# apschera2023uzk/MWR_fast_forward_operators_and_LBLs

Hardware: AMD Instinct MI355X
Metric: TB evaluations/sec (profile x channel x angle) (higher is better)
Workload: dtype f64

## Files before the change

mwr_fast_forward_operators_and_lbls_amd/csrc/mwrt_absorption.hip.h:

```cpp
#pragma once
#include "mwrt_math.hip.h"

namespace mwrt {

typedef const __attribute__((address_space(4))) LineMasks* cmasks;
__device__ __forceinline__ LineMasks load_masks(const LineMasks* table, int chunk) {
  const cmasks q = (cmasks)table + chunk;
  LineMasks lm;
  lm.o2_far = q->o2_far; lm.h2o_far = q->h2o_far; lm.h2o_none = q->h2o_none; lm.h2o_res = q->h2o_res; lm.h2o_sd = q->h2o_sd;
  lm.h2o_sdfar = q->h2o_sdfar; lm.h2o_sdint = q->h2o_sdint;
  lm.h2o_vfar = q->h2o_vfar; lm.o2_vfar = q->o2_vfar; lm.vf_u0 = q->vf_u0; lm.vf_h = q->vf_h; lm.vf_invh = q->vf_invh;
  return lm;
}

struct LevelState {
  double t;
  double p;
  double rho;
  double pdry;
};

__device__ __forceinline__ double goff_gratch_e(double tk, double rh) {
  const double LN10 = 2.302585092994045684;
  const double INV_LN10 = 0.434294481903251828;
// ... 122 lines not shown
  }
}
template <int NFC>
__device__ __forceinline__ void far_group_close(const double (&N)[NFC], const double (&D)[NFC], double (&sum)[NFC]) {
  double r[NFC];
#pragma unroll
  for (int j = 0; j < NFC; ++j) r[j] = __builtin_amdgcn_rcp(D[j]);
#pragma unroll
  for (int j = 0; j < NFC; ++j) r[j] = __builtin_fma(r[j], __builtin_fma(-D[j], r[j], 1.0), r[j]);
#pragma unroll
  for (int j = 0; j < NFC; ++j) sum[j] = N[j] * r[j];
}
template <int NFC, class Mask, class Setup>
__device__ __forceinline__ void far_groups_accumulate(const double* sfq, Mask m, Setup&& setup, double (&sum)[NFC]) {
  auto next_quad = [&](FarLine (&q)[4]) {
#pragma unroll
    for (int i = 0; i < 4; ++i) { setup(__builtin_ctzll((unsigned long long)m), q[i]); m &= m - Mask(1); }
    LDS_RELOAD_FENCE();
  };
  while (m) {
    double N[NFC], D[NFC];
    {
      FarLine q[4];
      next_quad(q);
      far_quad_fraction<NFC, true>(sfq, q[0], q[1], q[2], q[3], sum, N, D);
    }
    for (int g = 1; g < FAR_GROUP_QUADS && m; ++g) {
      FarLine q[4];
      next_quad(q);
      far_quad_fraction<NFC, false>(sfq, q[0], q[1], q[2], q[3], sum, N, D);
    }
    far_group_close<NFC>(N, D, sum);
  }
}

constexpr int VF_TERMS = 8;
__device__ __forceinline__ void vfar_add(const FarLine& fl, double u0, double h, double (&acc)[VF_TERMS]) {
  const double d0 = __builtin_fma(u0, u0 + fl.A2, fl.Bc);
  const double d1h = __builtin_fma(fl.A2, h, (2.0 * u0) * h);
  double rd = __builtin_amdgcn_rcp(d0);
  rd = __builtin_fma(rd, __builtin_fma(-d0, rd, 1.0), rd);
  const double a = -d1h * rd, b = (-(h * h)) * rd;
  double cm2 = __builtin_fma(fl.P, u0, fl.Q) * rd;
  double cm1 = __builtin_fma(a, cm2, (fl.P * h) * rd);
  acc[0] += cm2;
  acc[1] += cm1;
#pragma unroll
  for (int j = 2; j < VF_TERMS; ++j) {
    const double cj = __builtin_fma(a, cm1, b * cm2);
    acc[j] += cj;
    cm2 = cm1; cm1 = cj;
  }
}
template <int NFC>
__device__ __forceinline__ void vfar_eval(const double* sfq, double invh, double mu , const double (&acc)[VF_TERMS], double (&sum)[NFC]) {
  constexpr int G = (NFC % 7 == 0) ? 7 : ((NFC % 4 == 0) ? 4 : 2);
  static_assert(NFC % G == 0, "group width");
#pragma unroll
  for (int j0 = 0; j0 < NFC; j0 += G) {
    double x[G], p[G];
#pragma unroll
    for (int g = 0; g < G; ++g) { x[g] = __builtin_fma(sfq[2 * (j0 + g) + 1], invh, mu); p[g] = acc[VF_TERMS - 1]; }
#pragma unroll
    for (int k = VF_TERMS - 2; k >= 0; --k) {
#pragma unroll
      for (int g = 0; g < G; ++g) p[g] = __builtin_fma(p[g], x[g], acc[k]);
// ... 268 lines not shown
        if (wave_any(inner)) {
          const double r1 = inner ? sd_shape(d1) - q.base : 0.0;
          sum[j] = __builtin_fma(q.s, r1, sum[j]);
        }
      }
    }
  }
  const bool dry = !(L.rho > 0.0);
#pragma unroll
  for (int j = 0; j < NFC; ++j) {
    const double f2 = sfq[2 * j + 1];
    awet[j] = dry ? 0.0 : (3.183e-05 * den * sum[j] + con0) * f2;
  }
}

template <bool FUSED>
__device__ __forceinline__ double table_addend(double s) {
  if constexpr (FUSED) {
    double v;
    asm("v_mov_b64 %0, %1" : "=v"(v) : "s"(s));
    return v;
  } else {
    return s;
  }
}

struct O2Line {
  double c1, df2;
  double P, Q;
  double cc;
  double dnu;
};

template <int NFC, bool NODES = false, bool GROUPED = false>
__device__ __forceinline__ void dry_absorb(cmodel M, const LevelState& L, const double* sfq ,
                                           const LineMasks& lm, double (&adry)[NFC], unsigned long long excl = 0ull,
                                           const double* init_sum = nullptr, unsigned long long* failed = nullptr) {
  const double temp = L.t;
  const double pres = L.p;
  const double th = fdiv(300.0, temp);
  const double th1 = th - 1.0;
  const double lnth = flog(th);
  const double b = fexp(M->o2_x * lnth);
  const double preswv = fdiv(L.rho * temp, M->o2_pvap_div);
  const double presda = pres - preswv;
  const double den = 0.001 * (presda * b + M->o2_wv_factor * preswv * th);
  const double dens = 0.001 * (presda + M->o2_wv_factor * preswv) * th;
  const double dfnr = M->o2_wb300 * den;
  const double pe2 = den * den;
  const bool second = M->o2_mix_mode != 0;
  const double ymul = second ? den : 0.001 * pres * b;
  const bool line1_dens = !second && M->o2_line1_dens;

  double sum[NFC];
#pragma unroll
  for (int j = 0; j < NFC; ++j) sum[j] = init_sum ? init_sum[j] : 0.0;

  long long be_prev = -1;
  double ebe = 1.0;
  auto line_setup = [&](int k) -> O2Line {
    const auto& R = M->o2r[k];
    if constexpr (GROUPED) asm volatile("" :: "s"(R.be), "s"(R.w300), "s"(R.y0), "s"(R.y1));
    const double y = ymul * __builtin_fma(R.y1, th1, table_addend<GROUPED>(R.y0));
    double dnu = 0.0, gfac = 1.0;
    if (second) {
      dnu = pe2 * __builtin_fma(R.dnu1, th1, table_addend<GROUPED>(R.dnu0));
      gfac = __builtin_fma(pe2, __builtin_fma(R.g1, th1, table_addend<GROUPED>(R.g0)), 1.0);
    }
    const double df = R.w300 * ((k == 0 && line1_dens) ? dens : den);
    const long long be_bits = __builtin_bit_cast(long long, R.be);
    if (be_bits != be_prev) { ebe = fexp(-R.be * th1); be_prev = be_bits; }
    const double str = R.s300rf2 * ebe;
    O2Line q;
    q.dnu = dnu;
    q.c1 = R.f + dnu;
    q.df2 = df * df;
    const double a = (str * df) * gfac;
    const double cb = q.c1 * (str * y);
    q.cc = __builtin_fma(q.c1, q.c1, q.df2);
    q.P = a + cb;
    q.Q = q.cc * (a - cb);
    return q;
  };

  const int nl = M->n_o2;
  const unsigned long long all = o2_lines_all(nl) & ~excl;
  unsigned long long near = ~lm.o2_far & all;
  const unsigned long long setA = (MWRT_ABLATE & 1) ? 0ull : o2_far_set(lm, all);
  const unsigned long long setV = o2_vfar_set(lm, setA, NODES);
  const unsigned long long setQ = o2_quad_set(lm, setA, NODES);
  const unsigned long long leftA = lowest_bits(setQ, __builtin_popcountll(setQ) & 3);
  const unsigned long long leftP = (__builtin_popcountll(leftA) >= 2) ? lowest_bits(leftA, 2) : 0ull;
  near |= leftA & ~leftP;
  auto far_setup = [&](int k, FarLine& fl) {
    const O2Line q = line_setup(k);
    double P = q.P, Q = q.Q;
    if (!NODES && second && !wave_all(fabs(q.dnu) < FAR_SHIFT_GHZ)) { near |= 1ull << k; P = 0.0; Q = 0.0; }
    fl.P = P; fl.Q = Q;
    fl.A2 = 2.0 * __builtin_fma(-q.c1, q.c1, q.df2);
    fl.Bc = q.cc * q.cc;
  };
  if (setV) {
    double acc[VF_TERMS];
#pragma unroll
    for (int j = 0; j < VF_TERMS; ++j) acc[j] = 0.0;
    for (unsigned long long m = setV; m; m &= m - 1ull) {
      FarLine q;
      far_setup(__builtin_ctzll(m), q);
      vfar_add(q, lm.vf_u0, lm.vf_h, acc);
    }
    LDS_RELOAD_FENCE();
    vfar_eval<NFC>(sfq, lm.vf_invh, -lm.vf_u0 * lm.vf_invh, acc, sum);
  }
  if constexpr (GROUPED) far_groups_accumulate<NFC>(sfq, setQ & ~leftA, far_setup, sum);
  else for (unsigned long long m = setQ & ~leftA; m;) {
    FarLine q0, q1, q2, q3;
    far_setup(__builtin_ctzll(m), q0); m &= m - 1ull;
    far_setup(__builtin_ctzll(m), q1); m &= m - 1ull;
    far_setup(__builtin_ctzll(m), q2); m &= m - 1ull;
    far_setup(__builtin_ctzll(m), q3); m &= m - 1ull;
    LDS_RELOAD_FENCE();
    far_quad_accumulate<NFC>(sfq, q0, q1, q2, q3, sum);
  }
  if (leftP) {
    FarLine q0, q1;
    unsigned long long m = leftP;
    far_setup(__builtin_ctzll(m), q0); m &= m - 1ull;
    far_setup(__builtin_ctzll(m), q1);
    LDS_RELOAD_FENCE();
    far_pair_accumulate<NFC>(sfq, q0, q1, sum);
  }
  if (MWRT_ABLATE & 1) near = 0ull;
  be_prev = -1;
  for (unsigned long long m = near; m; m &= m - 1ull) {
    const int k = __builtin_ctzll(m);
    const O2Line q = line_setup(k);
    LDS_RELOAD_FENCE();
#pragma unroll
    for (int j = 0; j < NFC; ++j) {
      const double f = sfq[2 * j], f2 = sfq[2 * j + 1];
      const double d1 = f - q.c1;
      const double d2 = f + q.c1;
      const double D1 = __builtin_fma(d1, d1, q.df2);
      const double D2 = __builtin_fma(d2, d2, q.df2);
      const double den12 = D1 * D2;
// ... 129 lines not shown
```

mwr_fast_forward_operators_and_lbls_amd/csrc/mwrt_fused.hip.h:

```cpp
#pragma once
#include "mwrt_absorption.hip.h"
#include "mwrt_layer.hip.h"

namespace mwrt {

__device__ __forceinline__ void blank_outputs(const FusedArgs& A, int64_t prof, int jbase, int nfc, int tid, int nthreads) {
  const double qnan = __builtin_nan("");
  const int nang = A.nang, nlev = A.nlev;
  for (int it = tid; it < nfc * nang; it += nthreads) {
    const int j = it / nang, a = it % nang;
    const int64_t o = (prof * nang + a) * A.nf + jbase + j;
    A.tb[o] = qnan;
    if (A.tbatm) A.tbatm[o] = qnan;
    if (A.tmr) A.tmr[o] = qnan;
    if (A.tauwet) A.tauwet[o] = qnan;
    if (A.taudry) A.taudry[o] = qnan;
    if (A.tauliq) A.tauliq[o] = qnan;
    if (A.tauice) A.tauice[o] = qnan;
  }
  if (A.taulay) for (int it = tid; it < nfc * nlev; it += nthreads)
    A.taulay[(prof * A.nf + jbase + it / nlev) * nlev + it % nlev] = qnan;
}

typedef const __attribute__((address_space(3))) double* ldoubles;
template <class Step>
__device__ __forceinline__ void rte_segment(const double* tau_seg, const double* bof_seg, int seglen, Step step) {
  ldoubles tp = (ldoubles)tau_seg, bp = (ldoubles)bof_seg;
  asm volatile("" : "+v"(tp), "+v"(bp));
  double t0 = tp[0], t1 = tp[1], b0 = bp[0], b1 = bp[1];
  for (int n = seglen >> 2; n > 0; --n) {
    const double t2 = tp[2], t3 = tp[3];
    step(t0, b0);
    const double b2 = bp[2], b3 = bp[3];
    step(t1, b1);
    t0 = tp[4]; t1 = tp[5];
    step(t2, b2);
    b0 = bp[4]; b1 = bp[5];
    step(t3, b3);
    tp += 4; bp += 4;
  }
  const int rest = seglen & 3;
  if (rest > 0) step(t0, b0);
  if (rest > 1) step(t1, b1);
  if (rest > 2) step(tp[2], bp[2]);
}

template <int NFC, int NFK, int MAXT, bool OPT = false, bool EXTRAS = false, bool ALPHA = false>
__global__ void __launch_bounds__(MAXT, (MAXT <= 256 ? (EXTRAS ? MWRT_MIN_WAVES : (ALPHA ? 4 : 3)) : 1))
k_tb_fused(const FusedArgs A) {
  constexpr int NPASS = (NFC + NFK - 1) / NFK;
  static_assert(NPASS <= 2, "LaunchGeom carries the split of two passes");
  extern __shared__ __attribute__((aligned(16))) double lds[];
  const int tid = threadIdx.x;
  const int lane = tid & (WAVE - 1);
  const int wave = tid / WAVE;
  const int nthreads = blockDim.x;
  const int nwaves = nthreads / WAVE;
  const int64_t prof = blockIdx.x;
  const int mi = (int)(prof / A.nprof_in);
  const int64_t pin = prof - mi * A.nprof_in;
  const int jbase = blockIdx.y * NFC;
  const int nfc = min(NFC, A.nf - jbase);
  const int nlev = A.nlev, nang = A.nang, ld = A.g.ldrow;
  const cmodel M = (cmodel)A.Ms[mi];
  const cdoubles cfrq = (cdoubles)A.frq;
  const cdoubles cam = (cdoubles)A.airmass;

  double* tau = lds;
  double* bof = tau + (size_t)NFK * ld;
  double* part = bof + (size_t)NFK * ld;
  double* scratch = part + (size_t)A.g.npart;
  double* edge = scratch + 16;
  auto row = [&](int j) -> double* { return (j < NFK ? tau + (size_t)j * ld : bof + (size_t)(j - NFK) * ld); };
  constexpr bool GROUPED = MAXT <= 512;
  constexpr bool PARK = !ALPHA && GROUPED;
  constexpr int GRP = 16;
  const int ngrp = nthreads / GRP;
// ... 49 lines not shown
      for (int j = 0; j < NFC; ++j) { awet[j] = 0.0; adry[j] = 0.0; }
    }
    if (active && bad) atomicOr(&s_flag, 1);
  }
  double denl = 0.0, deni = 0.0, o3n = 0.0;
  if constexpr (OPT) {
    if (A.denliq) denl = A.denliq[off];
    if (A.denice) deni = A.denice[off];
    if (A.o3n) o3n = A.o3n[off];
    if (active && (isnan(denl) || isnan(deni) || isnan(o3n))) atomicOr(&s_flag, 1);
  }
  __syncthreads();
  if (s_flag) {
    blank_outputs(A, prof, jbase, nfc, tid, nthreads);
    if (tid == 0) A.valid[prof] = 0;
    return;
  }

  if constexpr (!ALPHA) {
    const double e = goff_gratch_e(ti, rhi);
    const LevelState L = level_state(pi, ti, e);
    const LineMasks lm = load_masks(A.masks[mi], blockIdx.y);
    MWRT_STAMP(1);
    MWRT_SETPRIO(3);
    h2o_absorb<NFC, false, GROUPED>(M, L, sfq, lm, awet);
    if constexpr (PARK) {
      if (active) {
#pragma unroll
        for (int j = 0; j < NFC; ++j) row(j)[tid] = awet[j];
      }
    }
    MWRT_STAMP(2);
    MWRT_SETPRIO(2);
    dry_absorb<NFC, false, GROUPED>(M, L, sfq, lm, adry);
    MWRT_SETPRIO(1);
    MWRT_STAMP(3);
    if constexpr (OPT) {
      if (A.o3n) {
        LDS_RELOAD_FENCE();
        x_absorb<NFC>(M, A.t[off], A.p[off], A.o3n[off], sfq, adry);
      }
    }
  }
  if (lane == WAVE - 1) {
#pragma unroll
    for (int j = 0; j < NFC; ++j) {
      if constexpr (!PARK) edge[wave * 2 * NFC + j] = awet[j];
      edge[wave * 2 * NFC + NFC + j] = adry[j];
    }
  }
  __syncthreads();
  if constexpr (OPT) { LDS_RELOAD_FENCE(); zi = A.z[off]; ti = A.t[off]; }
  double tw[EXTRAS ? NFC : 1], td[NFC];
  bool neg = false;
  {
    const double z0 = A.z[pin * nlev];
    const double dz = (active && tid > 0) ? ((zi - z0) - (A.z[off - 1] - z0)) : 0.0;
    const bool seam = (lane == 0) && (wave > 0);
    const bool has_prev = active && tid > 0;
    [[maybe_unused]] ldoubles wrow = nullptr;
    [[maybe_unused]] double pw_next = 0.0, aw_next = 0.0;
    if constexpr (PARK) {
      wrow = (ldoubles)(tau + (has_prev ? tid - 1 : 0));
      asm volatile("" : "+v"(wrow));
      if (wave_live) { pw_next = wrow[0]; aw_next = wrow[1]; }
    }
    if (!wave_live) {
#pragma unroll
      for (int j = 0; j < NFC; ++j) { td[j] = 0.0; if constexpr (EXTRAS) tw[j] = 0.0; }
    } else
#pragma unroll
    for (int j = 0; j < NFC; ++j) {
#pragma clang fp contract(off)
      double aw, pw;
      if constexpr (PARK) {
        aw = aw_next; pw = pw_next;
        if (j + 1 < NFC) { wrow += ld; pw_next = wrow[0]; aw_next = wrow[1]; }
      } else {
        aw = awet[j];
        pw = __shfl_up(awet[j], 1, WAVE);
        if (seam) pw = edge[(wave - 1) * 2 * NFC + j];
      }
      double pd = __shfl_up(adry[j], 1, WAVE);
      if (seam) pd = edge[(wave - 1) * 2 * NFC + NFC + j];
      const double lw = layer_value(aw, pw, neg, has_prev), ld_ = layer_value(adry[j], pd, neg, has_prev);
// ... 139 lines not shown
        }
        __syncthreads();
        if (active) {
#pragma unroll
          for (int jj = 0; jj < NFK; ++jj) {
            const int j = h * NFK + jj;
            if (j < NFC) tau[jj * ld + tid] = ((tw[j] + td[j]) + tci[j]) + tl[j];
          }
        }
      }
    }
    __syncthreads();

    int nthin_all = 0;
    if (sorted) {
      const bool mine = tid < items;
      const int it = mine ? tid : 0;
      const int pr = div_small(it, nseg, A.g.magic_nseg[h]), seg = it - pr * nseg;
      const int jj = div_small(pr, nang, A.g.magic_nang), a = pr - jj * nang;
      const int lo = 1 + seg * seglen, hi = min(lo + seglen, nlev);
      float gm = 0.0f;
      for (int g = lo / GRP; g <= (hi - 1) / GRP; ++g) gm = fmaxf(gm, gmax[jj * ngrp + g]);
      const bool thin = mine && !((double)gm * cam[a] > EXP_SMALL_X);
      const unsigned long long bal = __ballot(thin);
      const int rank = __popcll(bal & ((1ull << lane) - 1ull));
      if (lane == 0) wcnt[wave] = __popcll(bal);
      __syncthreads();
      int before = 0, nthin = 0;
      for (int w = 0; w < nwaves; ++w) { const int c = wcnt[w]; nthin += c; if (w < wave) before += c; }
      if (mine) perm[thin ? before + rank : nthin + tid - (before + rank)] = (a << 11) | (jj << 7) | seg;
      nthin_all = nthin;
      __syncthreads();
    }
    for (int it0 = tid; it0 < items; it0 += nthreads) {
      int seg, jj, a;
      if (sorted) {
        const int key = perm[it0];
        seg = key & 127; jj = (key >> 7) & 15; a = key >> 11;
      } else {
        const int pr = div_small(it0, nseg, A.g.magic_nseg[h]);
        seg = it0 - pr * nseg; jj = div_small(pr, nang, A.g.magic_nang); a = pr - jj * nang;
      }
      const int it = (jj * nang + a) * nseg + seg;
      const double am = cam[a];
      const int lo = 1 + seg * seglen;
      const int hi = min(lo + seglen, nlev);
      const double* tj = tau + jj * ld;
      const double* bj = bof + jj * ld;
      const double* fr = nullptr;
      if constexpr (OPT) fr = A.amf ? A.amf + (pin * nang + a) * nlev : nullptr;
      double T = 1.0, B = 0.0;
      double bprev = (lo < nlev) ? bj[lo - 1] : 0.0;
      if (!sorted && !(OPT && fr) && nseg * seglen < ld) {
        const double cs = loop_invariant_vgpr(FEXP_SMALL_C0), ce = loop_invariant_vgpr(FEXP_C0);
        const double ct = loop_invariant_vgpr(FTANH_HALF_SMALL_C0);
        const double nam = -am;
        rte_segment(tj + lo, bj + lo, seglen, [&](double tz, double bi) {
          const double ntl = tz * nam;
          if (wave_all(fabs(ntl) <= EXP_SMALL_X)) {
            KEEP_BRANCH();
            const double E = fexp_small(ntl, cs);
            const double nth = ftanh_half_small(ntl, ct);
            B = __builtin_fma(__builtin_fma(bi, E, bprev) * T, -nth, B);
            T *= E;
          } else {
            KEEP_BRANCH();
            const double E = fexp(ntl, ce);
// ... 88 lines not shown
```

mwr_fast_forward_operators_and_lbls_amd/csrc/mwrt.hip:

```cpp
#include "mwrt_host.hip.h"
#include "mwrt_args.hip.h"
#include "mwrt_tl.hip.h"
#include "mwrt_ray.hip.h"
#include "mwrt_par.hip.h"
#include "mwrt_plan.h"

#include <cmath>
#include <cstddef>
#include <cstdio>
#include <cstdlib>
#include <cstring>
#include <string>
#include <vector>
#include <new>
#include <atomic>

using namespace mwrt;

namespace {
thread_local std::string g_err;
}

int mwrt::fail(int code, const std::string& msg) { g_err = msg; return code; }

// ... 66 lines not shown
size_t g_phase_cap = 0;
int phase_attach(FusedArgs* a, int64_t nprof, int nchunks, hipStream_t st) {
  const size_t phase_n = (size_t)nprof * 4 * 10;
  a->phase = nullptr;
  if (!std::getenv("MWRT_PHASE_DUMP") || nchunks != 1) return MWRT_OK;
  if (g_phase_cap < phase_n) { if (g_phase) (void)hipFree(g_phase); HIP_TRY(hipMalloc((void**)&g_phase, phase_n * 8)); g_phase_cap = phase_n; }
  HIP_TRY(hipMemsetAsync(g_phase, 0, phase_n * 8, st));
  a->phase = g_phase;
  return MWRT_OK;
}
int phase_dump(const FusedArgs& a, int64_t nprof, hipStream_t st) {
  if (!a.phase) return MWRT_OK;
  const size_t phase_n = (size_t)nprof * 4 * 10;
  std::vector<long long> h(phase_n);
  HIP_TRY(hipStreamSynchronize(st));
  HIP_TRY(hipMemcpy(h.data(), g_phase, phase_n * 8, hipMemcpyDeviceToHost));
  if (FILE* f = std::fopen(std::getenv("MWRT_PHASE_DUMP"), "wb")) { std::fwrite(h.data(), 8, phase_n, f); std::fclose(f); }
  return MWRT_OK;
}
#else
int phase_attach(FusedArgs*, int64_t, int, hipStream_t) { return MWRT_OK; }
int phase_dump(const FusedArgs&, int64_t, hipStream_t) { return MWRT_OK; }
#endif

int launch_fused(mwrt_context* c, int nfc, FusedArgs a, int64_t nprof, hipStream_t st, int variant) {
  int threads = lanes_for(a.nlev);
  if (variant == FUSED_FROM_ALPHA && threads < 256 && a.nang > 1) threads = 256;
  const int nchunks = (a.nf + nfc - 1) / nfc;
  size_t lds = 0;
  if (!plan_fused(c->lds_max, nfc, a.nlev, a.nf, a.nang, &a.g, &lds, threads))
    return fail(MWRT_ERR_UNSUPPORTED, "LDS budget exceeded (nlev x nang too large)");
  dim3 grid((unsigned)nprof , (unsigned)nchunks), block(threads);
  a.write_valid = nchunks == 1;
  if (!a.write_valid) HIP_TRY(hipMemsetAsync(a.valid, 1, (size_t)nprof, st));
  int rc = phase_attach(&a, nprof, nchunks, st); if (rc) return rc;
  rc = timed(c, st, [&] {
    switch (nfc) {
      case 8: return launch_fused_nfc8(a, grid, block, lds, st, variant);
      case 14: return launch_fused_nfc14(a, grid, block, lds, st, variant);
      default: return launch_fused_nfc16(a, grid, block, lds, st, variant);
    }
  });
  return rc ? rc : phase_dump(a, nprof, st);
}

int launch_absorb(mwrt_context* c, int nfc, const AbsorbArgs& a, int64_t nprof, hipStream_t st) {
  const int nchunks = (a.nf + nfc - 1) / nfc;
  dim3 grid((unsigned)nprof, (unsigned)nchunks), block(lanes_for(a.nlev));
  return timed(c, st, [&] {
    switch (nfc) {
      case 8: return launch_absorb_nfc8(a, grid, block, st);
      case 14: return launch_absorb_nfc14(a, grid, block, st);
      default: return launch_absorb_nfc16(a, grid, block, st);
    }
  });
}

int launch_windowed_absorption(mwrt_context* c, const mwrt_model* m, int64_t nprof, int nlev, const double* d_p, const double* d_t,
                               const double* d_rh, int nf, const double* frq, const double* dev_frq, double* d_awet,
                               double* d_adry, const TauOut* T, int threads, hipStream_t st) {
  DeviceCache::Blob b;
  const hipError_t e = c->win_cache.get(m->id, 0, frq, nf, c->stream, [&](std::vector<char>* host) {
    WindowSet ws;
    build_windows(m->h_desc, frq, nf, &ws);
    pack_windows(ws, nf, host);
    return (int)ws.wins.size();
// ... 241 lines not shown
int mwrt_version(void) { return MWRT_VERSION; }

size_t mwrt_model_desc_size(void) { return sizeof(mwrt_model_desc); }

int mwrt_device_count(void) {
  int n = 0;
  if (hipGetDeviceCount(&n) != hipSuccess) { (void)hipGetLastError(); return 0; }
  return n;
}

const char* mwrt_last_error(void) { return g_err.c_str(); }

int mwrt_create(int device_id, mwrt_context** out) {
  if (!out) return fail(MWRT_ERR_INVALID_ARGUMENT, "out is null");
  *out = nullptr;
  const int n = mwrt_device_count();
  if (n <= 0) return fail(MWRT_ERR_NO_DEVICE, "no HIP device: this library has no CPU path");
  if (device_id < 0 || device_id >= n) return fail(MWRT_ERR_INVALID_ARGUMENT, "device_id out of range");
  HIP_TRY(hipSetDevice(device_id));
  mwrt_context* c = new (std::nothrow) mwrt_context();
  if (!c) return fail(MWRT_ERR_OUT_OF_MEMORY, "host allocation failed");
  c->device = device_id;
  hipError_t e = hipStreamCreateWithFlags(&c->stream, hipStreamNonBlocking);
  if (e != hipSuccess) { delete c; return fail(MWRT_ERR_HIP, hipGetErrorString(e)); }
  int lds = 0;
  if (hipDeviceGetAttribute(&lds, hipDeviceAttributeMaxSharedMemoryPerBlock, device_id) == hipSuccess && lds > 0)
    c->lds_max = lds;
  int cus = 0;
  if (hipDeviceGetAttribute(&cus, hipDeviceAttributeMultiprocessorCount, device_id) == hipSuccess && cus > 0) c->num_cus = cus;
  if (const char* mb = std::getenv("MWRT_ALPHA_BATCH_MB")) {
    const long v = std::atol(mb);
    if (v > 0) c->alpha_batch_bytes = (size_t)v << 20;
  }
  *out = c;
  return MWRT_OK;
}

int mwrt_destroy(mwrt_context* c) {
  if (!c) return MWRT_OK;
  (void)hipSetDevice(c->device);
  (void)hipStreamSynchronize(c->stream);
  c->win_cache.release(); c->mask_cache.release();
  c->frq_cache.release(); c->am_cache.release(); c->elev_cache.release(); c->d_amf.release(); c->d_duct.release(); c->d_alpha.release();
  c->d_jac.release();
  c->d_par.release(); c->par_cache.release();
  c->d_in.release(); c->d_out.release();
  c->d_valid.release(); c->d_ex.release();
  for (DeviceHandle* h : c->handles_live) {
    (void)hipFree(h->d_blob);
    h->d_blob = nullptr; h->ctx = nullptr;
  }
  for (hipEvent_t e : c->ev0) (void)hipEventDestroy(e);
  for (hipEvent_t e : c->ev1) (void)hipEventDestroy(e);
  if (c->ws_event) (void)hipEventDestroy(c->ws_event);
  (void)hipStreamDestroy(c->stream);
  delete c;
  return MWRT_OK;
}

int mwrt_model_create(mwrt_context* c, const mwrt_model_desc* desc, mwrt_model** out) {
  if (!c || !desc || !out) return fail(MWRT_ERR_INVALID_ARGUMENT, "null argument");
  *out = nullptr;
  if (desc->n_h2o < 0 || desc->n_h2o > MWRT_MAX_H2O_LINES || desc->n_o2 < 0 || desc->n_o2 > MWRT_MAX_O2_LINES)
    return fail(MWRT_ERR_INVALID_ARGUMENT, "line counts out of range");
  if (desc->n_x < 0 || desc->n_x > MWRT_MAX_X_LINES) return fail(MWRT_ERR_INVALID_ARGUMENT, "extra-species line count out of range");
  HIP_TRY(hipSetDevice(c->device));
// ... 654 lines not shown
```

mwr_fast_forward_operators_and_lbls_amd/csrc/mwrt_args.hip.h:

```cpp
#pragma once
#include <hip/hip_runtime.h>
#include <stdint.h>
#include "../../include/mwrt.h"
#include "mwrt_plan.h"

#ifndef MWRT_PHASE_CLOCK
#define MWRT_PHASE_CLOCK 0
#endif

namespace mwrt {

constexpr double TAUMAX = 125.0;
constexpr double TRANS_MIN = 5.1664206328378610e-55;

struct O2Rec { double f, s300rf2, be, w300, y0, y1, g0, g1, dnu0, dnu1, pad[6]; };
struct H2ORec { double fl, s1, b2, w0, x, w0s, xs, sh, xh, shs, xhs, aair, aself, w2, pad[2]; };
struct ModelFlat : mwrt_model_desc {
  double o2_rf2[MWRT_MAX_O2_LINES];
  O2Rec o2r[MWRT_MAX_O2_LINES];
  H2ORec h2or[MWRT_MAX_H2O_LINES];
};
typedef const __attribute__((address_space(4))) ModelFlat* cmodel;
typedef const __attribute__((address_space(4))) double* cdoubles;

struct FusedArgs {
  const ModelFlat* Ms[MAX_MULTI];
  int64_t nprof_in;
  const double* z; const double* p; const double* t; const double* rh;
  const double* frq;
  const double* airmass;
  double* tb;
  uint8_t* valid;
  double* tbatm; double* tmr; double* tauwet; double* taudry;
  double* taulay;
  int nlev, nf, nang;
  int write_valid;
  LaunchGeom g;
  const double* denliq; const double* denice;
  const double* amf;
  const uint8_t* duct;
  double* tauliq; double* tauice;
  const double* awet_in; const double* adry_in;
  const LineMasks* masks[MAX_MULTI];
  const double* o3n;
#if MWRT_PHASE_CLOCK
  long long* phase;
#endif
};

struct TauOut {
  const double* z;
  double* tau;
  uint8_t* valid;
  int fpitch;
};

struct AbsorbArgs {
  const ModelFlat* M;
  const double* p; const double* t; const double* rh;
  const double* frq;
  double* awet; double* adry;
  int nlev, nf;
  TauOut T;
  const LineMasks* masks;
};

struct AbsorbWinArgs {
  const ModelFlat* M;
  const double* p; const double* t; const double* rh;
  const double* frq;
  const WinDesc* win;
  const double* lagrange;
  const double* lagrange_h;
  const LineMasks* masks;
  const double* lag_sd;
  double* awet; double* adry;
  int nlev, nf;
// ... 47 lines not shown
```

mwr_fast_forward_operators_and_lbls_amd/csrc/mwrt_host.hip.h:

```cpp
#pragma once
#include <hip/hip_runtime.h>
#include "../../include/mwrt.h"

#include <cstring>
#include <string>
#include <vector>

namespace mwrt {

int fail(int code, const std::string& msg);

#define HIP_TRY(expr)                                                                        \
  do {                                                                                       \
    hipError_t e_ = (expr);                                                                  \
    if (e_ != hipSuccess)                                                                    \
      return fail(e_ == hipErrorOutOfMemory ? MWRT_ERR_OUT_OF_MEMORY : MWRT_ERR_HIP,         \
                  std::string(#expr) + ": " + hipGetErrorString(e_));                        \
  } while (0)

struct DevBuf {
  void* p = nullptr;
  size_t cap = 0;
  hipError_t reserve(size_t bytes) {
    if (bytes <= cap) return hipSuccess;
// ... 43 lines not shown
      entries_.erase(entries_.begin() + (long)lru);
    }
    Entry ne{model, tag, std::vector<double>(key, key + n), nullptr, count, 0};
    hipError_t e = hipMalloc((void**)&ne.dev, host.empty() ? 1 : host.size());
    if (e != hipSuccess) return e;
    e = hipMemcpyAsync(ne.dev, host.data(), host.size(), hipMemcpyHostToDevice, copy_stream);
    if (e == hipSuccess) e = hipStreamSynchronize(copy_stream);
    if (e != hipSuccess) { (void)hipFree(ne.dev); return e; }
    ne.stamp = ++clock_;
    entries_.push_back(std::move(ne));
    *out = Blob{entries_.back().dev, count};
    return hipSuccess;
  }
  std::vector<Entry> entries_;
  size_t capacity_;
  unsigned long clock_ = 0;
};

struct DeviceHandle {
  mwrt_context* ctx = nullptr;
  void* d_blob = nullptr;
};

}

struct mwrt_context {
  int device = 0;
  hipStream_t stream = nullptr;
  int lds_max = 65536;
  int num_cus = 256;
  mwrt::DeviceCache frq_cache{32}, am_cache{32}, elev_cache{32};
  int absorption_mode = 0;
  int chunk_width = 0;
  mwrt::DeviceCache win_cache{16};
  mwrt::DeviceCache mask_cache{64};
  mwrt::DevBuf d_amf, d_duct;
  mwrt::DevBuf d_alpha;
  size_t alpha_batch_bytes = (size_t)4 << 30;
  hipEvent_t ws_event = nullptr;
  hipStream_t ws_stream = nullptr;
  bool ws_used = false;
  mwrt::DevBuf d_jac;
  mwrt::DevBuf d_par;
  mwrt::DeviceCache par_cache{32};
  mwrt::DevBuf d_in, d_out, d_valid, d_ex;
  bool timing = false;
  std::vector<hipEvent_t> ev0, ev1;
  long ev_count = 0;
  std::vector<mwrt::DeviceHandle*> handles_live;
};

namespace mwrt {

constexpr int TIMING_RING = 512;

inline hipStream_t resolve_stream(const mwrt_context* c, void* stream) {
  if (!stream) return c->stream;
  if (stream == MWRT_STREAM_LEGACY) return (hipStream_t) nullptr;
  return (hipStream_t)stream;
}

template <class F> int timed(mwrt_context* c, hipStream_t st, F launch) {
  if (c->timing) (void)hipEventRecord(c->ev0[c->ev_count % TIMING_RING], st);
  const hipError_t e = launch();
  if (c->timing) { (void)hipEventRecord(c->ev1[c->ev_count % TIMING_RING], st); c->ev_count++; }
  HIP_TRY(e);
// ... 5 lines not shown
```

mwr_fast_forward_operators_and_lbls_amd/csrc/mwrt_math.hip.h:

```cpp
#pragma once
#include "mwrt_args.hip.h"

namespace mwrt {

__device__ __forceinline__ int div_small(int n, int d, unsigned magic) {
  return d == 1 ? n : (int)__umulhi((unsigned)n, magic);
}

#ifndef MWRT_EXACT_DIV
#define MWRT_EXACT_DIV 0
#endif
#ifndef MWRT_ABLATE
#define MWRT_ABLATE 0
#endif
#ifndef MWRT_NO_SETPRIO
#define MWRT_NO_SETPRIO 0
#endif
#if MWRT_NO_SETPRIO
#define MWRT_SETPRIO(n) do { } while (0)
#else
#define MWRT_SETPRIO(n) __builtin_amdgcn_s_setprio(n)
#endif
#if MWRT_PHASE_CLOCK
#define MWRT_STAMP(k) do { if (A.phase && lane == 0) A.phase[((int64_t)blockIdx.x * 4 + wave) * 10 + (k)] = (long long)wall_clock64(); } while (0)
// ... 73 lines not shown
  const double s = num * r;
  const double z = s * s;
  const double p = two_atanh_tail(z);
  const double ed = (double)e;
  const double lm = __builtin_fma(s * z, p, s + s);
  return __builtin_fma(ed, 6.93147180369123816490e-01, __builtin_fma(ed, 1.90821492927058770002e-10, lm));
#endif
}

constexpr double EXP_SMALL_X = 0.125;
constexpr double FEXP_SMALL_C0 = 2.756514908613403e-06;
__device__ __forceinline__ double fexp_small(double x, double c0 = FEXP_SMALL_C0) {
  double p = c0;
  MWRT_FMA_SC(p, x, 2.4810200365624755e-05);
  MWRT_FMA_SC(p, x, 0.00019841269076602318);
  MWRT_FMA_SC(p, x, 0.001388888804772704);
  MWRT_FMA_SC(p, x, 0.008333333333357229);
  MWRT_FMA_SC(p, x, 0.04166666666692954);
  MWRT_FMA_SC(p, x, 0.16666666666666666);
  MWRT_FMA_SC(p, x, 0.4999999999999999);
  p = __builtin_fma(p, x, 1.0);
  return __builtin_fma(p, x, 1.0);
}

constexpr double FTANH_HALF_SMALL_C0 = 4.257889640378761e-05;
__device__ __forceinline__ double ftanh_half_small(double x, double c0 = FTANH_HALF_SMALL_C0) {
  const double u = x * x;
  double p = c0;
  MWRT_FMA_SC(p, u, -0.0004216256671577941);
  MWRT_FMA_SC(p, u, 0.004166666662552237);
  MWRT_FMA_SC(p, u, -0.04166666666666466);
  p = __builtin_fma(p, u, 0.5);
  return p * x;
}

constexpr double EXP_TINY_X = 0.015625;
__device__ __forceinline__ double fexp_tiny(double x) {
  double p = 1.3888888888888889e-03;
  MWRT_FMA_SC(p, x, 8.3333333333333332e-03);
  MWRT_FMA_SC(p, x, 4.1666666666666664e-02);
  MWRT_FMA_SC(p, x, 1.6666666666666666e-01);
  p = __builtin_fma(p, x, 0.5);
  p = __builtin_fma(p, x, 1.0);
  return __builtin_fma(p, x, 1.0);
}
__device__ __forceinline__ double ftanh_half_tiny(double x) {
  const double u = x * x;
  double p = -4.2162698412698413e-04;
  MWRT_FMA_SC(p, u, 4.1666666666666666e-03);
  MWRT_FMA_SC(p, u, -4.1666666666666664e-02);
  p = __builtin_fma(p, u, 0.5);
  return p * x;
}

typedef unsigned long long wmask;
__device__ __forceinline__ bool wave_all(bool p) { return __builtin_amdgcn_ballot_w64(!p) == 0ull; }
__device__ __forceinline__ bool wave_any(bool p) { return __builtin_amdgcn_ballot_w64(p) != 0ull; }
__device__ __forceinline__ wmask wballot(bool p) { return __builtin_amdgcn_ballot_w64(p); }
template <class... B>
__device__ __forceinline__ bool wave_all_of(B... b) { return (wballot(b) & ...) == wballot(true); }

__device__ __forceinline__ float row16_max(float m) {
  m = fmaxf(m, __int_as_float(__builtin_amdgcn_update_dpp(0, __float_as_int(m), 0x128, 0xf, 0xf, false)));
  m = fmaxf(m, __int_as_float(__builtin_amdgcn_update_dpp(0, __float_as_int(m), 0x124, 0xf, 0xf, false)));
  m = fmaxf(m, __int_as_float(__builtin_amdgcn_update_dpp(0, __float_as_int(m), 0x122, 0xf, 0xf, false)));
  m = fmaxf(m, __int_as_float(__builtin_amdgcn_update_dpp(0, __float_as_int(m), 0x121, 0xf, 0xf, false)));
// ... 104 lines not shown
```

Baseline: 1.031 billion.

## Fold O2 near-line and nonresonant tail into grouped rational-fraction accumulation

In the grouped fused kernel, the O2 near lines, leftover far lines and the nonresonant term are merged into the open far-group numerator/denominator fraction, so one division per group replaces per-line divisions. The last partially filled far group is left open so tail members can join it, and a separate path computes the final dry absorption and returns early. The fused kernel also reloads z, t and the liquid and ice densities from memory after the barrier when parking, to reduce register pressure. Risks include extra numeric range issues from multiplying denominators and more code in the kernel.

```diff
diff --git a/mwr_fast_forward_operators_and_lbls_amd/csrc/mwrt_absorption.hip.h b/mwr_fast_forward_operators_and_lbls_amd/csrc/mwrt_absorption.hip.h
--- a/mwr_fast_forward_operators_and_lbls_amd/csrc/mwrt_absorption.hip.h
+++ b/mwr_fast_forward_operators_and_lbls_amd/csrc/mwrt_absorption.hip.h
@@ -178,6 +178,58 @@
     }
     far_group_close<NFC>(N, D, sum);
   }
+}
+
+constexpr int TAIL_GROUP_MEMBERS = 4 * FAR_GROUP_QUADS;
+__device__ __forceinline__ void tail_merge(double& n, double& d, double num, double den) {
+  fma_in_place(n, den, num * d);
+  d *= den;
+}
+template <int NFC, class Mask, class Setup>
+__device__ __forceinline__ int far_groups_open(const double* sfq, Mask m, Setup&& setup, double (&sum)[NFC], double (&N)[NFC], double (&D)[NFC]) {
+  auto next_quad = [&](FarLine (&q)[4]) {
+#pragma unroll
+    for (int i = 0; i < 4; ++i) { setup(__builtin_ctzll((unsigned long long)m), q[i]); m &= m - Mask(1); }
+    LDS_RELOAD_FENCE();
+  };
+  int open = 0;
+  while (m) {
+    {
+      FarLine q[4];
+      next_quad(q);
+      far_quad_fraction<NFC, true>(sfq, q[0], q[1], q[2], q[3], sum, N, D);
+    }
+    int g = 1;
+    for (; g < FAR_GROUP_QUADS && m; ++g) {
+      FarLine q[4];
+      next_quad(q);
+      far_quad_fraction<NFC, false>(sfq, q[0], q[1], q[2], q[3], sum, N, D);
+    }
+    if (m) far_group_close<NFC>(N, D, sum);
+    else open = g;
+  }
+  return open;
+}
+template <int NFC>
+__device__ __forceinline__ void tail_group_begin(const double (&sum)[NFC], double (&N)[NFC], double (&D)[NFC]) {
+#pragma unroll
+  for (int j = 0; j < NFC; ++j) { N[j] = sum[j]; D[j] = 1.0; }
+}
+template <int NFC>
+__device__ __forceinline__ int tail_start(int quads, int members, double (&sum)[NFC], double (&N)[NFC], double (&D)[NFC]) {
+  if (quads > 0 && quads + (members + 3) / 4 <= FAR_GROUP_QUADS) return 4 * (FAR_GROUP_QUADS - quads);
+  if (quads > 0) far_group_close<NFC>(N, D, sum);
+  tail_group_begin<NFC>(sum, N, D);
+  return TAIL_GROUP_MEMBERS;
+}
+template <int NFC>
+__device__ __forceinline__ void tail_member(int& room, double (&sum)[NFC], double (&N)[NFC], double (&D)[NFC]) {
+  if (room == 0) {
+    far_group_close<NFC>(N, D, sum);
+    tail_group_begin<NFC>(sum, N, D);
+    room = TAIL_GROUP_MEMBERS;
+  }
+  --room;
 }
 
 constexpr int VF_TERMS = 8;
@@ -512,7 +564,7 @@
   double dnu;
 };
 
-template <int NFC, bool NODES = false, bool GROUPED = false>
+template <int NFC, bool NODES = false, bool GROUPED = false, bool TAILS = false>
 __device__ __forceinline__ void dry_absorb(cmodel M, const LevelState& L, const double* sfq ,
                                            const LineMasks& lm, double (&adry)[NFC], unsigned long long excl = 0ull,
                                            const double* init_sum = nullptr, unsigned long long* failed = nullptr) {
@@ -571,7 +623,8 @@
   const unsigned long long setQ = o2_quad_set(lm, setA, NODES);
   const unsigned long long leftA = lowest_bits(setQ, __builtin_popcountll(setQ) & 3);
   const unsigned long long leftP = (__builtin_popcountll(leftA) >= 2) ? lowest_bits(leftA, 2) : 0ull;
-  near |= leftA & ~leftP;
+  static_assert(!TAILS || (GROUPED && !NODES), "the tail rides in the fused kernel's groups");
+  near |= TAILS ? leftA : leftA & ~leftP;
   auto far_setup = [&](int k, FarLine& fl) {
     const O2Line q = line_setup(k);
     double P = q.P, Q = q.Q;
@@ -591,6 +644,48 @@
     }
     LDS_RELOAD_FENCE();
     vfar_eval<NFC>(sfq, lm.vf_invh, -lm.vf_u0 * lm.vf_invh, acc, sum);
+  }
+  if constexpr (TAILS) {
+    double N[NFC], D[NFC];
+    const int quads = far_groups_open<NFC>(sfq, setQ & ~leftA, far_setup, sum, N, D);
+    if (MWRT_ABLATE & 1) near = 0ull;
+    int room = tail_start<NFC>(quads, __builtin_popcountll(near) + 1, sum, N, D);
+    be_prev = -1;
+    for (unsigned long long m = near; m; m &= m - 1ull) {
+      const int k = __builtin_ctzll(m);
+      const O2Line q = line_setup(k);
+      LDS_RELOAD_FENCE();
+      tail_member<NFC>(room, sum, N, D);
+#pragma unroll
+      for (int j = 0; j < NFC; ++j) {
+        const double f = sfq[2 * j], f2 = sfq[2 * j + 1];
+        const double d1 = f - q.c1;
+        const double d2 = f + q.c1;
+        const double D1 = __builtin_fma(d1, d1, q.df2);
+        const double D2 = __builtin_fma(d2, d2, q.df2);
+        tail_merge(N[j], D[j], __builtin_fma(f2, q.P, q.Q), D1 * D2);
+      }
+    }
+    double th1l = th1, denl = den;
+    asm volatile("" : "+v"(th1l), "+v"(denl));
+    const double thl = th1l + 1.0, dfnrl = M->o2_wb300 * denl;
+    const double nrq = fdiv(0.5 * M->o2_nonres * dfnrl, thl);
+    const double dfnr2 = dfnrl * dfnrl;
+    LDS_RELOAD_FENCE();
+    tail_member<NFC>(room, sum, N, D);
+#pragma unroll
+    for (int j = 0; j < NFC; ++j) tail_merge(N[j], D[j], nrq, sfq[2 * j + 1] + dfnr2);
+    far_group_close<NFC>(N, D, sum);
+    const double scale2 = 2.0 * M->o2_coef * presda * thl * thl * thl;
+    const double pn2 = M->n2_ptot ? pres : L.pdry;
+    const double n2c = M->n2_n * M->n2_l * pn2 * pn2 * fexp(M->n2_m * lnth);
+#pragma unroll
+    for (int j = 0; j < NFC; ++j) {
+      const double f2 = sfq[2 * j + 1];
+      const double o2 = fmax(scale2 * (sum[j] * f2), 0.0);
+      adry[j] = o2 + n2c * sfq[2 * NFC + 2 + j] * f2;
+    }
+    return;
   }
   if constexpr (GROUPED) far_groups_accumulate<NFC>(sfq, setQ & ~leftA, far_setup, sum);
   else for (unsigned long long m = setQ & ~leftA; m;) {
diff --git a/mwr_fast_forward_operators_and_lbls_amd/csrc/mwrt_fused.hip.h b/mwr_fast_forward_operators_and_lbls_amd/csrc/mwrt_fused.hip.h
--- a/mwr_fast_forward_operators_and_lbls_amd/csrc/mwrt_fused.hip.h
+++ b/mwr_fast_forward_operators_and_lbls_amd/csrc/mwrt_fused.hip.h
@@ -158,7 +158,7 @@
     }
     MWRT_STAMP(2);
     MWRT_SETPRIO(2);
-    dry_absorb<NFC, false, GROUPED>(M, L, sfq, lm, adry);
+    dry_absorb<NFC, false, GROUPED, GROUPED>(M, L, sfq, lm, adry);
     MWRT_SETPRIO(1);
     MWRT_STAMP(3);
     if constexpr (OPT) {
@@ -176,7 +176,11 @@
     }
   }
   __syncthreads();
-  if constexpr (OPT) { LDS_RELOAD_FENCE(); zi = A.z[off]; ti = A.t[off]; }
+  if constexpr (OPT || PARK) { LDS_RELOAD_FENCE(); zi = A.z[off]; ti = A.t[off]; }
+  if constexpr (OPT && PARK) {
+    if (A.denliq) denl = A.denliq[off];
+    if (A.denice) deni = A.denice[off];
+  }
   double tw[EXTRAS ? NFC : 1], td[NFC];
   bool neg = false;
   {
```

New measurement: 1.040 billion, median of 6. About the same (+0.8%).

## Process two RTE segment items per thread with interleaved exp/tanh evaluation

Applied to the files above, without the earlier changes.

Adds a paired path to the fused kernel's segment-wise radiative transfer loop. Each thread now handles two work items (itA and itA+nthreads) at once and interleaves their recurrence steps, with paired polynomial exp/tanh and reciprocal routines. The aim is more instruction-level parallelism to hide FMA and LDS latency in the serial per-layer dependency chain. The cost is higher register pressure and extra branch combinations for thin versus general layers. It is on by default and can be disabled with MWRT_K2_PAIRS=0.

```diff
diff --git a/mwr_fast_forward_operators_and_lbls_amd/csrc/mwrt.hip b/mwr_fast_forward_operators_and_lbls_amd/csrc/mwrt.hip
--- a/mwr_fast_forward_operators_and_lbls_amd/csrc/mwrt.hip
+++ b/mwr_fast_forward_operators_and_lbls_amd/csrc/mwrt.hip
@@ -122,6 +122,7 @@
     return fail(MWRT_ERR_UNSUPPORTED, "LDS budget exceeded (nlev x nang too large)");
   dim3 grid((unsigned)nprof , (unsigned)nchunks), block(threads);
   a.write_valid = nchunks == 1;
+  a.k2_pairs = c->k2_pairs;
   if (!a.write_valid) HIP_TRY(hipMemsetAsync(a.valid, 1, (size_t)nprof, st));
   int rc = phase_attach(&a, nprof, nchunks, st); if (rc) return rc;
   rc = timed(c, st, [&] {
@@ -429,6 +430,8 @@
     const long v = std::atol(mb);
     if (v > 0) c->alpha_batch_bytes = (size_t)v << 20;
   }
+  if (const char* kp = std::getenv("MWRT_K2_PAIRS"))
+    c->k2_pairs = !(kp[0] == '0' && kp[1] == '\0');
   *out = c;
   return MWRT_OK;
 }
diff --git a/mwr_fast_forward_operators_and_lbls_amd/csrc/mwrt_args.hip.h b/mwr_fast_forward_operators_and_lbls_amd/csrc/mwrt_args.hip.h
--- a/mwr_fast_forward_operators_and_lbls_amd/csrc/mwrt_args.hip.h
+++ b/mwr_fast_forward_operators_and_lbls_amd/csrc/mwrt_args.hip.h
@@ -43,6 +43,7 @@
   const double* awet_in; const double* adry_in;
   const LineMasks* masks[MAX_MULTI];
   const double* o3n;
+  int k2_pairs;
 #if MWRT_PHASE_CLOCK
   long long* phase;
 #endif
diff --git a/mwr_fast_forward_operators_and_lbls_amd/csrc/mwrt_fused.hip.h b/mwr_fast_forward_operators_and_lbls_amd/csrc/mwrt_fused.hip.h
--- a/mwr_fast_forward_operators_and_lbls_amd/csrc/mwrt_fused.hip.h
+++ b/mwr_fast_forward_operators_and_lbls_amd/csrc/mwrt_fused.hip.h
@@ -43,6 +43,74 @@
   if (rest > 0) step(t0, b0);
   if (rest > 1) step(t1, b1);
   if (rest > 2) step(tp[2], bp[2]);
+}
+
+template <class Step>
+__device__ __forceinline__ void rte_segment2(const double* tauA, const double* bofA, const double* tauB, const double* bofB,
+                                             int seglen, Step step) {
+  ldoubles tpA = (ldoubles)tauA, bpA = (ldoubles)bofA, tpB = (ldoubles)tauB, bpB = (ldoubles)bofB;
+  asm volatile("" : "+v"(tpA), "+v"(bpA), "+v"(tpB), "+v"(bpB));
+  double tA0 = tpA[0], tA1 = tpA[1], bA0 = bpA[0], bA1 = bpA[1];
+  double tB0 = tpB[0], tB1 = tpB[1], bB0 = bpB[0], bB1 = bpB[1];
+  for (int n = seglen >> 2; n > 0; --n) {
+    const double tA2 = tpA[2], tA3 = tpA[3], tB2 = tpB[2], tB3 = tpB[3];
+    step(tA0, bA0, tB0, bB0);
+    const double bA2 = bpA[2], bA3 = bpA[3], bB2 = bpB[2], bB3 = bpB[3];
+    step(tA1, bA1, tB1, bB1);
+    tA0 = tpA[4]; tA1 = tpA[5]; tB0 = tpB[4]; tB1 = tpB[5];
+    step(tA2, bA2, tB2, bB2);
+    bA0 = bpA[4]; bA1 = bpA[5]; bB0 = bpB[4]; bB1 = bpB[5];
+    step(tA3, bA3, tB3, bB3);
+    tpA += 4; bpA += 4; tpB += 4; bpB += 4;
+  }
+  const int rest = seglen & 3;
+  if (rest > 0) step(tA0, bA0, tB0, bB0);
+  if (rest > 1) step(tA1, bA1, tB1, bB1);
+  if (rest > 2) step(tpA[2], bpA[2], tpB[2], bpB[2]);
+}
+
+__device__ __forceinline__ void k2_step_thin(double ntl, double bi, double& bprev, double& T, double& B, double cs, double ct) {
+  const double E = fexp_small(ntl, cs);
+  const double nth = ftanh_half_small(ntl, ct);
+  B = __builtin_fma(__builtin_fma(bi, E, bprev) * T, -nth, B);
+  T *= E;
+  bprev = bi;
+}
+__device__ __forceinline__ void k2_step_general(double ntl, double bi, double& bprev, double& T, double& B, double ce) {
+  const double E = fexp(ntl, ce);
+  const double lay = fdiv1(__builtin_fma(bi, E, bprev), 1.0 + E);
+  B = __builtin_fma(lay * T, 1.0 - E, B);
+  T *= E;
+  bprev = bi;
+}
+__device__ __forceinline__ void k2_step_thin2(double ntlA, double biA, double& bprevA, double& TA, double& BA,
+                                              double ntlB, double biB, double& bprevB, double& TB, double& BB,
+                                              double cs, double ct) {
+  double EA, EB, nthA, nthB;
+  fexp_tanh_small2(ntlA, ntlB, cs, ct, EA, EB, nthA, nthB);
+  const double sA = __builtin_fma(biA, EA, bprevA) * TA, sB = __builtin_fma(biB, EB, bprevB) * TB;
+  BA = __builtin_fma(sA, -nthA, BA); BB = __builtin_fma(sB, -nthB, BB);
+  TA *= EA; TB *= EB;
+  bprevA = biA; bprevB = biB;
+}
+__device__ __forceinline__ void k2_step_general2(double ntlA, double biA, double& bprevA, double& TA, double& BA,
+                                                 double ntlB, double biB, double& bprevB, double& TB, double& BB, double ce) {
+#if MWRT_EXACT_DIV
+  k2_step_general(ntlA, biA, bprevA, TA, BA, ce);
+  k2_step_general(ntlB, biB, bprevB, TB, BB, ce);
+#else
+  double EA, EB;
+  fexp2(ntlA, ntlB, ce, EA, EB);
+  const double dA = 1.0 + EA, dB = 1.0 + EB;
+  double rA = __builtin_amdgcn_rcp(dA), rB = __builtin_amdgcn_rcp(dB);
+  const double nA = __builtin_fma(biA, EA, bprevA), nB = __builtin_fma(biB, EB, bprevB);
+  const double eA = __builtin_fma(-dA, rA, 1.0), eB = __builtin_fma(-dB, rB, 1.0);
+  rA = __builtin_fma(rA, eA, rA); rB = __builtin_fma(rB, eB, rB);
+  const double layA = nA * rA, layB = nB * rB;
+  BA = __builtin_fma(layA * TA, 1.0 - EA, BA); BB = __builtin_fma(layB * TB, 1.0 - EB, BB);
+  TA *= EA; TB *= EB;
+  bprevA = biA; bprevB = biB;
+#endif
 }
 
 template <int NFC, int NFK, int MAXT, bool OPT = false, bool EXTRAS = false, bool ALPHA = false>
@@ -382,7 +450,61 @@
       nthin_all = nthin;
       __syncthreads();
     }
-    for (int it0 = tid; it0 < items; it0 += nthreads) {
+    int it_first = tid;
+    if constexpr (MAXT <= 512) {
+      if (A.k2_pairs && !sorted && !(OPT && A.amf) && nseg * seglen < ld) {
+        const double cs = loop_invariant_vgpr(FEXP_SMALL_C0), ce = loop_invariant_vgpr(FEXP_C0);
+        const double ct = loop_invariant_vgpr(FTANH_HALF_SMALL_C0);
+        int base = 0;
+        for (; base + nthreads < items; base += 2 * nthreads) {
+          const int itA = base + tid;
+          const bool hasB = itA + nthreads < items;
+          const int itB = hasB ? itA + nthreads : itA;
+          const wmask maskB = wballot(hasB);
+          const int prA = div_small(itA, nseg, A.g.magic_nseg[h]), segA = itA - prA * nseg;
+          const int jjA = div_small(prA, nang, A.g.magic_nang), aA = prA - jjA * nang;
+          const int prB = div_small(itB, nseg, A.g.magic_nseg[h]), segB = itB - prB * nseg;
+          const int jjB = div_small(prB, nang, A.g.magic_nang), aB = prB - jjB * nang;
+          const int loA = 1 + segA * seglen, loB = 1 + segB * seglen;
+          const double* tjA = tau + jjA * ld;
+          const double* bjA = bof + jjA * ld;
+          const double* tjB = tau + jjB * ld;
+          const double* bjB = bof + jjB * ld;
+          double TA = 1.0, BA = 0.0, TB = 1.0, BB = 0.0;
+          double bprevA = (loA < nlev) ? bjA[loA - 1] : 0.0;
+          double bprevB = (loB < nlev) ? bjB[loB - 1] : 0.0;
+          const double namA = -cam[aA], namB = -cam[aB];
+          rte_segment2(tjA + loA, bjA + loA, tjB + loB, bjB + loB, seglen, [&](double tzA, double biA, double tzB, double biB) {
+            const double ntlA = tzA * namA, ntlB = tzB * namB;
+            const bool thinA = wave_all(fabs(ntlA) <= EXP_SMALL_X);
+            const bool thinB = (wballot(!(fabs(ntlB) <= EXP_SMALL_X)) & maskB) == 0ull;
+            if (thinA) {
+              if (thinB) {
+                KEEP_BRANCH();
+                k2_step_thin2(ntlA, biA, bprevA, TA, BA, ntlB, biB, bprevB, TB, BB, cs, ct);
+              } else {
+                KEEP_BRANCH();
+                k2_step_thin(ntlA, biA, bprevA, TA, BA, cs, ct);
+                k2_step_general(ntlB, biB, bprevB, TB, BB, ce);
+              }
+            } else {
+              if (thinB) {
+                KEEP_BRANCH();
+                k2_step_general(ntlA, biA, bprevA, TA, BA, ce);
+                k2_step_thin(ntlB, biB, bprevB, TB, BB, cs, ct);
+              } else {
+                KEEP_BRANCH();
+                k2_step_general2(ntlA, biA, bprevA, TA, BA, ntlB, biB, bprevB, TB, BB, ce);
+              }
+            }
+          });
+          part[2 * itA + 0] = BA; part[2 * itA + 1] = TA;
+          if (hasB) { part[2 * itB + 0] = BB; part[2 * itB + 1] = TB; }
+        }
+        it_first = base + tid;
+      }
+    }
+    for (int it0 = it_first; it0 < items; it0 += nthreads) {
       int seg, jj, a;
       if (sorted) {
         const int key = perm[it0];
diff --git a/mwr_fast_forward_operators_and_lbls_amd/csrc/mwrt_host.hip.h b/mwr_fast_forward_operators_and_lbls_amd/csrc/mwrt_host.hip.h
--- a/mwr_fast_forward_operators_and_lbls_amd/csrc/mwrt_host.hip.h
+++ b/mwr_fast_forward_operators_and_lbls_amd/csrc/mwrt_host.hip.h
@@ -99,6 +99,7 @@
   mwrt::DeviceCache frq_cache{32}, am_cache{32}, elev_cache{32};
   int absorption_mode = 0;
   int chunk_width = 0;
+  bool k2_pairs = true;
   mwrt::DeviceCache win_cache{16};
   mwrt::DeviceCache mask_cache{64};
   mwrt::DevBuf d_amf, d_duct;
diff --git a/mwr_fast_forward_operators_and_lbls_amd/csrc/mwrt_math.hip.h b/mwr_fast_forward_operators_and_lbls_amd/csrc/mwrt_math.hip.h
--- a/mwr_fast_forward_operators_and_lbls_amd/csrc/mwrt_math.hip.h
+++ b/mwr_fast_forward_operators_and_lbls_amd/csrc/mwrt_math.hip.h
@@ -129,6 +129,45 @@
   MWRT_FMA_SC(p, u, -0.04166666666666466);
   p = __builtin_fma(p, u, 0.5);
   return p * x;
+}
+
+#define MWRT_FMA_SC2(pa, ra, pb, rb, c) do { MWRT_FMA_SC(pa, ra, c); MWRT_FMA_SC(pb, rb, c); } while (0)
+__device__ __forceinline__ void fexp_tanh_small2(double xa, double xb, double ce, double ct, double& Ea, double& Eb,
+                                                 double& tha, double& thb) {
+  const double ua = xa * xa, ub = xb * xb;
+  double pa = ce, pb = ce, qa = ct, qb = ct;
+  MWRT_FMA_SC2(pa, xa, pb, xb, 2.4810200365624755e-05);
+  MWRT_FMA_SC2(qa, ua, qb, ub, -0.0004216256671577941);
+  MWRT_FMA_SC2(pa, xa, pb, xb, 0.00019841269076602318);
+  MWRT_FMA_SC2(qa, ua, qb, ub, 0.004166666662552237);
+  MWRT_FMA_SC2(pa, xa, pb, xb, 0.001388888804772704);
+  MWRT_FMA_SC2(qa, ua, qb, ub, -0.04166666666666466);
+  MWRT_FMA_SC2(pa, xa, pb, xb, 0.008333333333357229);
+  qa = __builtin_fma(qa, ua, 0.5); qb = __builtin_fma(qb, ub, 0.5);
+  MWRT_FMA_SC2(pa, xa, pb, xb, 0.04166666666692954);
+  tha = qa * xa; thb = qb * xb;
+  MWRT_FMA_SC2(pa, xa, pb, xb, 0.16666666666666666);
+  MWRT_FMA_SC2(pa, xa, pb, xb, 0.4999999999999999);
+  pa = __builtin_fma(pa, xa, 1.0); pb = __builtin_fma(pb, xb, 1.0);
+  Ea = __builtin_fma(pa, xa, 1.0); Eb = __builtin_fma(pb, xb, 1.0);
+}
+__device__ __forceinline__ void fexp2(double xa, double xb, double c0, double& Ea, double& Eb) {
+  const double ka = __builtin_rint(xa * 1.4426950408889634074), kb = __builtin_rint(xb * 1.4426950408889634074);
+  double ra = __builtin_fma(ka, -6.93147180369123816490e-01, xa), rb = __builtin_fma(kb, -6.93147180369123816490e-01, xb);
+  ra = __builtin_fma(ka, -1.90821492927058770002e-10, ra); rb = __builtin_fma(kb, -1.90821492927058770002e-10, rb);
+  double pa = c0, pb = c0;
+  MWRT_FMA_SC2(pa, ra, pb, rb, 2.762032742826824e-07);
+  MWRT_FMA_SC2(pa, ra, pb, rb, 2.75572680728901e-06);
+  MWRT_FMA_SC2(pa, ra, pb, rb, 2.4801520792572694e-05);
+  MWRT_FMA_SC2(pa, ra, pb, rb, 0.00019841269863303223);
+  MWRT_FMA_SC2(pa, ra, pb, rb, 0.0013888888917538296);
+  MWRT_FMA_SC2(pa, ra, pb, rb, 0.008333333333330011);
+  MWRT_FMA_SC2(pa, ra, pb, rb, 0.04166666666662348);
+  MWRT_FMA_SC2(pa, ra, pb, rb, 0.16666666666666669);
+  MWRT_FMA_SC2(pa, ra, pb, rb, 0.5000000000000001);
+  pa = __builtin_fma(pa, ra, 1.0); pb = __builtin_fma(pb, rb, 1.0);
+  pa = __builtin_fma(pa, ra, 1.0); pb = __builtin_fma(pb, rb, 1.0);
+  Ea = __builtin_amdgcn_ldexp(pa, (int)ka); Eb = __builtin_amdgcn_ldexp(pb, (int)kb);
 }
 
 constexpr double EXP_TINY_X = 0.015625;
```

Result: no change. 1.034 billion before, 1.034 billion after (-0.1%).
